# LRMPUT/PUTSLAM

Measured on AMD Instinct MI355X. Metric: frame-pairs/s (match+RANSAC+Kabsch), 640x480 @ 2000 kpts, higher is better.
Workload: dtype f32; 1 GPU; BASELINE configs[2]: TUM fr1/desk-style synthetic sequence, 500 frames = 499 frame pairs per step per GPU, 2000 kpts/frame, 256-bit descriptors, Hamming BF + cross-check -> depth filter -> H=4096 3-pt Umeyama hypotheses (fixed) scored with errorVersion 1 -> refit; inputs resident in HBM; kpts=2000, hypotheses=4096, world_size=1, force_dist=False, estimator=fixed, streams=4, join=end, submit=ps_batch_queue_submit: whole batches to the library's chains in turn, matcher_kernel=mfma-fused, score_kernel=fast, hw_queues=4, accepted_pairs=499

## Files before the change

### profiles/isa_mix.py

```python
#!/usr/bin/env python3
import json
import os
import re
import subprocess
import sys
import tempfile
from collections import Counter

ROOT = os.path.dirname(os.path.dirname(os.path.abspath(__file__)))
FLAGS = ["--offload-arch=gfx950", "-O3", "-ffp-contract=off", "-std=c++17", "-mllvm", "-amdgpu-mfma-vgpr-form",
         "-fno-slp-vectorize", "-mllvm", "-disable-vector-combine", "-S", "--cuda-device-only",
         "-I", os.path.join(ROOT, "include"), "-I", os.path.join(ROOT, "putslam_amd", "csrc")]


def asm_of(src, td, name):
    out = os.path.join(td, name)
    subprocess.check_call(["/opt/rocm/bin/hipcc"] + FLAGS + ["-o", out, src], stderr=subprocess.DEVNULL)
    return open(out).read()


def body_of(s, sym):
    a = s.index("\n" + sym)
    return s[a:s.index(".Lfunc_end", a)]


def blocks_of(body):
    parts = re.split(r"\n(\.LBB\d+_\d+:|; %bb\.\d+:)", body)
    return [(parts[i], parts[i + 1]) for i in range(1, len(parts), 2)]


def valu(txt):
    return Counter(re.sub(r"_e(32|64)$", "", l.split()[0]) for l in txt.split("\n") if l.strip().startswith("v_"))


def summary(c):
    n = sum(c.values())
    pk = sum(v for k, v in c.items() if k.startswith("v_pk_"))
    return {"valu": n, "packed": pk, "mix": dict(c)}


def main():
    out = {"source": "hipcc -S of putslam_amd/csrc/ps_capi.hip and profiles/microbench/prologue_isa.hip with the library's flags"}
    with tempfile.TemporaryDirectory() as td:
        s = asm_of(os.path.join(ROOT, "putslam_amd", "csrc", "ps_capi.hip"), td, "capi.s")
        pro = asm_of(os.path.join(ROOT, "profiles", "microbench", "prologue_isa.hip"), td, "pro.s")
    for mode in (1, 2):
        for kind, label in ((0, "stage0"), (1, "stage1")):
            bl = blocks_of(body_of(s, "_ZN5psdev20ps_ransac_score_fastILi%dELb1ELi%dELb0EE" % (mode, kind)))
            evals = [valu(t) for _, t in bl if "v_addc_co_u32" in t and t.count("v_pk_") >= 8]
            pre = [valu(t) for _, t in bl if "v_addc_co_u32" not in t and t.count("v_pk_") >= 12 and "ds_" not in t]
            e = {"unit": "(hypothesis, match) evaluation per wave"}
            if evals:
                per_block = max(1, evals[0]["v_addc_co_u32"])
                sm = summary(evals[0])
                e.update({"valu": sm["valu"] / per_block, "packed": sm["packed"] / per_block,
                          "mix": {k: v / per_block for k, v in sm["mix"].items()}})
                e["evaluations_per_block"] = per_block
                e["evaluation_blocks"] = len(evals)
            if pre and kind == 1:
                e["pretest"] = dict(summary(pre[0]), unit="TWO matches, one direction, per wave")
            out["ps_ransac_score_fast<%d> %s" % (mode, label)] = e
    for mode in (0, 4):
        bl = blocks_of(body_of(s, "_ZN5psdev22ps_ransac_score_euclidILi%dELi1ELb0EE" % mode))
        hot = [(t.count("clamp"), valu(t)) for _, t in bl if "clamp" in t]
        hot.sort(key=lambda x: -x[0])
        steps = hot[0][0]
        out["ps_ransac_score_euclid<%d>" % mode] = dict(summary(hot[0][1]), unit="block of %d packed steps = %d matches per wave" % (steps, 2 * steps),
                                                        valu_per_match=sum(hot[0][1].values()) / (2.0 * steps),
                                                        packed_per_match=sum(v for k, v in hot[0][1].items() if k.startswith("v_pk_")) / (2.0 * steps))
    for mode in (0, 1, 2, 4):
        bl = blocks_of(body_of(s, "_ZN5psdev15ps_ransac_scoreILi%dEE" % mode))
        loops = {}
        for n, t in bl:
            first = t.split("\n", 1)[0]
            m = re.search(r"Header=(BB\d+_\d+)", first)
            hdr = m.group(1) if m else (n.strip(".:L") if "Loop Header" in first else None)
            if hdr:
                loops.setdefault(hdr, []).append(t)
        best = max(loops.values(), key=lambda ts: sum(t.count("s_load_dwordx4") for t in ts))
        hot = Counter()
        for t in best:
            if "v_div_scale_f32" not in t and "v_cvt_f64_f32" not in t:
                hot += valu(t)
        per = max(1, "\n".join(best).count("s_load_dwordx4") // 2) if mode in (0, 4) else 1
        out["ps_ransac_score<%d>" % mode] = dict(summary(hot), unit="match loop body per wave (%d matches)" % per, valu_per_match=sum(hot.values()) / per)
    bl = blocks_of(body_of(s, "_ZN5psdev21ps_hamming_mfma_fusedILi4EE"))
    mf = max((t for _, t in bl), key=lambda t: t.count("v_mfma"))
    c = valu(mf)
    nm = sum(v for k, v in c.items() if k.startswith("v_mfma"))
    for k in [k for k in c if k.startswith("v_mfma")]:
        del c[k]
    out["ps_hamming_mfma_fused<4>"] = dict(summary(c), unit="query tile x 4 train tiles per wave (4096 distances)", mfma_per_unit=nm)
    bl = blocks_of(body_of(s, "_ZN5psdev13ps_hamming_nnILi2EE"))
    hb = max((t for _, t in bl), key=lambda t: t.count("v_bcnt"))
    c = valu(hb)
    out["ps_hamming_nn"] = dict(summary(c), unit="block of %d descriptor pairs per wave" % (c["v_bcnt_u32_b32"] // 8),
                                valu_per_pair=sum(c.values()) / (c["v_bcnt_u32_b32"] / 8.0))
    for sym in ("k_sample", "k_umeyama", "k_inverse"):
        bl = blocks_of(body_of(pro, sym + ":"))
        tot, loop = Counter(), Counter()
        for n, t in bl:
            c = valu(t)
            tot += c
            if "in Loop:" in t.split("\n", 1)[0] or "Loop Header" in t.split("\n", 1)[0]:
                loop += c
        full_div = tot["v_div_fixup_f32"]
        out["prologue " + sym] = {"static_valu": sum(tot.values()), "static_valu_in_loops": sum(loop.values()),
                                  "full_ieee_divisions": full_div, "reciprocal_chains": tot["v_rcp_f32"],
                                  "square_roots": tot["v_sqrt_f32"], "moves_and_selects": tot["v_mov_b32"] + tot["v_cndmask_b32"],
                                  "note": "static: both sides of every window check are in the count (short form AND the '/' fallback); "
                                          "the dynamic figure per wavefront is measured (sq_counters_by_grid.json, stage 0's models-only launch)"}
    with open(os.path.join(ROOT, "profiles", "isa_mix.json"), "w") as f:
        json.dump(out, f, indent=1)
    for k, v in out.items():
        if isinstance(v, dict):
            print(k, {a: b for a, b in v.items() if a not in ("mix", "note", "pretest")}, ("pretest %s" % {a: b for a, b in v["pretest"].items() if a != "mix"}) if "pretest" in v else "")


if __name__ == "__main__":
    main()
```

### putslam_amd/csrc/ps_matcher_mfma.h

```cpp
#pragma once

#include "ps_kernels.h"

namespace psdev {

typedef int v4i_t __attribute__((ext_vector_type(4)));
typedef int v8i_t __attribute__((ext_vector_type(8)));
typedef float v16f_t __attribute__((ext_vector_type(16)));

constexpr int kTileRows = 32;
constexpr int kTileU4 = 256;
constexpr int kWavesPerWG = kBlock / 64;

PS_HD constexpr uint32_t fp4_word(uint32_t w, int j, uint32_t sign = 0x88888888u, uint32_t fill = 0x66666666u)
{
    return (sign & (w << (3 - j))) | (~sign & fill);
}
constexpr bool fp4_word_checks(uint32_t w)
{
    for (int j = 0; j < 4; ++j) {
        const uint32_t o = fp4_word(w, j);
        if ((o & 0x77777777u) != 0x66666666u) return false;
        for (int i = 0; i < 8; ++i)
            if (((o >> (4 * i + 3)) & 1u) != ((w >> (4 * i + j)) & 1u)) return false;
    }
    return true;
}
constexpr bool fp4_single_bits_check()
{
    for (int b = 0; b < 32; ++b) {
        int hits = 0;
        for (int j = 0; j < 4; ++j)
            for (int i = 0; i < 8; ++i)
                if ((fp4_word(1u << b, j) >> (4 * i + 3)) & 1u) hits += (4 * i + j == b) ? 1 : 100;
        if (hits != 1 || !fp4_word_checks(1u << b) || !fp4_word_checks(~(1u << b))) return false;
    }
    return true;
}
static_assert(fp4_single_bits_check(), "every descriptor bit is the sign of exactly one nibble");
static_assert(fp4_word_checks(0u) && fp4_word_checks(0xFFFFFFFFu) && fp4_word_checks(0x80000001u) &&
                  fp4_word_checks(0xDEADBEEFu) && fp4_word_checks(0x01234567u) && fp4_word_checks(0xA5A5C3C3u) &&
                  fp4_word_checks(0x0F0F00FFu) && fp4_word_checks(0x13579BDFu),
              "fp4_word: sign of nibble i of dword j = bit 4 i + j, magnitude 0b110");
static_assert(fp4_word(0u, 0) == 0x66666666u && fp4_word(0xFFFFFFFFu, 2) == 0xEEEEEEEEu && fp4_word(0x10u, 0) == 0x000000E0u + 0x66666606u,
              "fp4_word: 0 -> +4.0, 1 -> -4.0");
PS_D v4i_t fp4_from_dword(uint32_t w)
{
    v4i_t r;
    r.x = (int)fp4_word(w, 0);
    r.y = (int)fp4_word(w, 1);
    r.z = (int)fp4_word(w, 2);
    r.w = (int)fp4_word(w, 3);
    return r;
}

PS_D int tile_row(int reg, int h) { return (reg & 3) + 8 * (reg >> 2) + 4 * h; }

__global__ __launch_bounds__(kBlock) void ps_expand_query_fp4(const uint32_t *__restrict__ desc,
                                                              const int32_t *__restrict__ nkpts,
                                                              const int32_t *__restrict__ pairs, int cap, int fstride, int tpf,
                                                              int chunks, uint4 *__restrict__ Xq,
                                                              uint32_t *__restrict__ keysInit)
{
    const int p = (int)(blockIdx.x / (unsigned)chunks), chunk = (int)(blockIdx.x % (unsigned)chunks);
    if (keysInit)
        for (int t = chunk * kBlock + threadIdx.x; t < cap; t += chunks * kBlock) keysInit[(size_t)p * cap + t] = kNoKey;
    const int fq = pairs[2 * p];
    const int nq = nkpts[fq];
    const uint32_t *__restrict__ q32 = desc + (size_t)fq * fstride;
    uint4 *__restrict__ out = Xq + (size_t)p * tpf * kTileU4;
    const int o = threadIdx.x, s = o >> 6, h = (o >> 5) & 1, r = o & 31;
    for (int tile = chunk; tile < tpf; tile += chunks) {
        const int row = tile * kTileRows + r;
        v4i_t e = {0, 0, 0, 0};
        if (row < nq) e = fp4_from_dword(q32[(size_t)row * 8 + 2 * s + h]);
        out[(size_t)tile * kTileU4 + o] = make_uint4((uint32_t)e.x, (uint32_t)e.y, (uint32_t)e.z, (uint32_t)e.w);
    }
}

PS_D v16f_t mfma_fp4(const v4i_t &a, const v4i_t &b, const v16f_t &c)
{
    const v8i_t a8 = __builtin_shufflevector(a, a, 0, 1, 2, 3, -1, -1, -1, -1);
    const v8i_t b8 = __builtin_shufflevector(b, b, 0, 1, 2, 3, -1, -1, -1, -1);
    return __builtin_amdgcn_mfma_scale_f32_32x32x64_f8f6f4(a8, b8, c, 4, 4, 0, 0, 0, 0);
}

PS_D v16f_t mfma_fp4s(const v4i_t &a, const v4i_t &b, const v16f_t &c)
{
    const v8i_t a8 = __builtin_shufflevector(a, a, 0, 1, 2, 3, -1, -1, -1, -1);
    const v8i_t b8 = __builtin_shufflevector(b, b, 0, 1, 2, 3, -1, -1, -1, -1);
    return __builtin_amdgcn_mfma_scale_f32_32x32x64_f8f6f4(a8, b8, c, 4, 4, 0, (int)0x88888888u, 0, (int)0x7F7F7F7Fu);
}

PS_D int fbits(float f) { return __builtin_bit_cast(int, f); }
PS_D int imax3(int a, int b, int c) { return max(max(a, b), c); }
PS_D int max16(const v16f_t &d)
{
    int m = imax3(fbits(d[0]), fbits(d[1]), fbits(d[2]));
    m = imax3(m, fbits(d[3]), fbits(d[4]));
    m = imax3(m, fbits(d[5]), fbits(d[6]));
    m = imax3(m, fbits(d[7]), fbits(d[8]));
    m = imax3(m, fbits(d[9]), fbits(d[10]));
    m = imax3(m, fbits(d[11]), fbits(d[12]));
    m = imax3(m, fbits(d[13]), fbits(d[14]));
    return max(m, fbits(d[15]));
}

constexpr float kMfmaNoRow = -1.0e30f;
constexpr int kMfmaBias = 8223;
constexpr float kMfmaBase = 8388608.0f;

#ifndef PS_MFMA_WAVES
#define PS_MFMA_WAVES 1
#endif
template <int TT>
__global__ __launch_bounds__(kBlock, PS_MFMA_WAVES) void ps_hamming_mfma(const uint32_t *__restrict__ desc,
                                                          const int32_t *__restrict__ nkpts,
                                                          const int32_t *__restrict__ pairs, int cap, int fstride, int tpf,
                                                          int groups, int qsplit, const uint4 *__restrict__ Xq,
                                                          uint32_t *__restrict__ keys)
{
    const unsigned perPair = (unsigned)(groups * qsplit);
    const unsigned L = xcd_remap(blockIdx.x, gridDim.x);
    const int p = (int)(L / perPair);
    const int inner = (int)(L - (unsigned)p * perPair);
    const int g = inner / qsplit, qs = inner - g * qsplit;
    const int fq = pairs[2 * p], ft = pairs[2 * p + 1];
    const int nq = nkpts[fq], nt = nkpts[ft];
    if (g * (kWavesPerWG * TT * kTileRows) >= nt) return;
    const int tid = threadIdx.x, lane = tid & 63, wave = tid >> 6;
    const int r = lane & 31, h = lane >> 5;
    const int tile0 = (g * kWavesPerWG + wave) * TT;
    const int nqTiles = (nq + kTileRows - 1) / kTileRows;
    const int T0 = (int)(((long long)nqTiles * qs) / qsplit), T1 = (int)(((long long)nqTiles * (qs + 1)) / qsplit);

    const uint32_t *__restrict__ t32 = desc + (size_t)ft * fstride;
    v4i_t B[TT][4];
#pragma unroll
    for (int i = 0; i < TT; ++i) {
        int t = (tile0 + i) * kTileRows + r;
        t = t < nt ? t : nt - 1;
#pragma unroll
        for (int s = 0; s < 4; ++s) B[i][s] = fp4_from_dword(t32[(size_t)t * 8 + 2 * s + h]);
    }
    v16f_t C;
#pragma unroll
    for (int reg = 0; reg < 16; ++reg) C[reg] = kMfmaBase + (float)(kMfmaBias - 4096 - tile_row(reg, h));
    int best[TT], bestT[TT];
#pragma unroll
    for (int i = 0; i < TT; ++i) {
        best[i] = 0;
        bestT[i] = 0;
    }

    const uint4 *__restrict__ xq = Xq + (size_t)p * tpf * kTileU4;
    uint4 an[4];
    if (T0 < T1) {
#pragma unroll
        for (int s = 0; s < 4; ++s) an[s] = xq[(size_t)T0 * kTileU4 + s * 64 + lane];
    }
    for (int T = T0; T < T1; ++T) {
        v4i_t A[4];
#pragma unroll
        for (int s = 0; s < 4; ++s) {
            A[s].x = (int)an[s].x; A[s].y = (int)an[s].y; A[s].z = (int)an[s].z; A[s].w = (int)an[s].w;
        }
        if (T + 1 < T1) {
#pragma unroll
            for (int s = 0; s < 4; ++s) an[s] = xq[(size_t)(T + 1) * kTileU4 + s * 64 + lane];
        }
        v16f_t Cin = C;
        if (T * kTileRows + kTileRows > nq) {
#pragma unroll
            for (int reg = 0; reg < 16; ++reg)
                if (T * kTileRows + tile_row(reg, h) >= nq) Cin[reg] = kMfmaNoRow;
        }
#pragma unroll
        for (int i = 0; i < TT; ++i) {
            v16f_t acc = mfma_fp4(A[0], B[i][0], Cin);
            acc = mfma_fp4(A[1], B[i][1], acc);
            acc = mfma_fp4(A[2], B[i][2], acc);
            acc = mfma_fp4(A[3], B[i][3], acc);
            const int m = max16(acc);
            if (m > (best[i] | 31)) {
                best[i] = m;
                bestT[i] = T;
            }
        }
    }
#pragma unroll
    for (int i = 0; i < TT; ++i) {
        const int t = (tile0 + i) * kTileRows + r;
        uint32_t key = kNoKey;
        if (best[i] > 0) {
            const int v = kMfmaBias - (best[i] & 0x7FFFFF);
            key = ((uint32_t)(v >> 5) << 16) | (uint32_t)(bestT[i] * kTileRows + (v & 31));
        }
        const uint32_t other = (uint32_t)__shfl_xor((int)key, 32, 64);
        key = other < key ? other : key;
        if (h == 0 && t < nt) {
            if (qsplit == 1)
                keys[(size_t)p * cap + t] = key;
            else
                atomicMin(&keys[(size_t)p * cap + t], key);
        }
    }
}

constexpr int kFuseChunk = 4;

template <int TT>
__global__ __launch_bounds__(kBlock, PS_MFMA_WAVES) void ps_hamming_mfma_fused(const uint32_t *__restrict__ desc,
                                                                const int32_t *__restrict__ nkpts,
                                                                const int32_t *__restrict__ pairs, int cap, int fstride, int tpf,
                                                                int groups, int qsplit, uint32_t *__restrict__ keys)
{
    __shared__ uint4 s_a[2][kFuseChunk][kTileU4];
    const unsigned perPair = (unsigned)(groups * qsplit);
    const unsigned L = xcd_remap(blockIdx.x, gridDim.x);
    const int p = (int)(L / perPair);
    const int inner = (int)(L - (unsigned)p * perPair);
    const int g = inner / qsplit, qs = inner - g * qsplit;
    const int fq = pairs[2 * p], ft = pairs[2 * p + 1];
    const int nq = nkpts[fq], nt = nkpts[ft];
    if (g * (kWavesPerWG * TT * kTileRows) >= nt) return;
    const int tid = threadIdx.x, lane = tid & 63, wave = tid >> 6;
    const int r = lane & 31, h = lane >> 5;
    const int tile0 = (g * kWavesPerWG + wave) * TT;
    const int nqTiles = (nq + kTileRows - 1) / kTileRows;
    const int T0 = (int)(((long long)nqTiles * qs) / qsplit), T1 = (int)(((long long)nqTiles * (qs + 1)) / qsplit);

    const uint32_t *__restrict__ t32 = desc + (size_t)ft * fstride;
    v4i_t B[TT][4];
#pragma unroll
    for (int i = 0; i < TT; ++i) {
        int t = (tile0 + i) * kTileRows + r;
        t = t < nt ? t : nt - 1;
#pragma unroll
        for (int s = 0; s < 4; ++s) B[i][s] = fp4_from_dword(t32[(size_t)t * 8 + 2 * s + h]);
    }
    v16f_t C;
#pragma unroll
    for (int reg = 0; reg < 16; ++reg) C[reg] = kMfmaBase + (float)((1 << 21) + 31 - tile_row(reg, h));
    int rel[TT];
#pragma unroll
    for (int i = 0; i < TT; ++i) rel[i] = 0;

    const uint32_t *__restrict__ q32 = desc + (size_t)fq * fstride;
    const int es = tid >> 6, eh = (tid >> 5) & 1, er = tid & 31;
    const int lastT = (nq & (kTileRows - 1)) ? nqTiles - 1 : -1;
    const bool hasPartial = lastT >= T0 && lastT < T1;
    const int Tm = hasPartial ? lastT : T1;
    const int nFull = (Tm - T0) / kFuseChunk;
    const int rem = (Tm - T0) - nFull * kFuseChunk;
    const int nTail = rem + (hasPartial ? 1 : 0);
    const int nChunks = nFull + (nTail > 0 ? 1 : 0);
    const uint32_t *__restrict__ qp = q32 + ((size_t)T0 * kTileRows + er) * 8 + 2 * es + eh;
    auto load_chunk = [&](int k, uint32_t (&W)[kFuseChunk]) {
        if (k < nFull) {
#pragma unroll
            for (int j = 0; j < kFuseChunk; ++j) W[j] = qp[j * (kTileRows * 8)];
            qp += kFuseChunk * kTileRows * 8;
        } else {
#pragma unroll
            for (int j = 0; j < kFuseChunk; ++j) {
                W[j] = 0;
                if (j < nTail && (T0 + nFull * kFuseChunk + j) * kTileRows + er < nq) W[j] = qp[j * (kTileRows * 8)];
            }
        }
    };
    uint32_t kSign = 0x88888888u, kFill = 0x66666666u;
    asm volatile("" : "+s"(kSign), "+v"(kFill));
    auto expand_chunk = [&](int buf, const uint32_t (&W)[kFuseChunk]) {
#pragma unroll
        for (int j = 0; j < kFuseChunk; ++j)
            s_a[buf][j][tid] = make_uint4(fp4_word(W[j], 0, kSign, kFill), fp4_word(W[j], 1, kSign, kFill),
                                          fp4_word(W[j], 2, kSign, kFill), fp4_word(W[j], 3, kSign, kFill));
    };
    auto tile_body = [&](const uint4 *__restrict__ tile, const v16f_t &Cin) {
        v4i_t A[4];
#pragma unroll
        for (int s = 0; s < 4; ++s) {
            const uint4 a = tile[s * 64 + lane];
            A[s].x = (int)a.x; A[s].y = (int)a.y; A[s].z = (int)a.z; A[s].w = (int)a.w;
        }
#pragma unroll
        for (int i = 0; i < TT; ++i) {
            v16f_t acc = mfma_fp4s(A[0], B[i][0], Cin);
            acc = mfma_fp4s(A[1], B[i][1], acc);
            acc = mfma_fp4s(A[2], B[i][2], acc);
            acc = mfma_fp4s(A[3], B[i][3], acc);
            int m = imax3(rel[i], fbits(acc[0]), fbits(acc[1]));
#pragma unroll
            for (int e = 2; e < 16; e += 2) m = imax3(m, fbits(acc[e]), fbits(acc[e + 1]));
            rel[i] = m + kTileRows;
        }
    };
    uint32_t W[kFuseChunk] = {0, 0, 0, 0};
    if (nChunks > 0) {
        load_chunk(0, W);
        expand_chunk(0, W);
    }
    if (nChunks > 1) load_chunk(1, W);
    __syncthreads();
    for (int k = 0; k < nFull; ++k) {
        expand_chunk((k + 1) & 1, W);
        if (k + 2 < nChunks) load_chunk(k + 2, W);
#pragma unroll 1
        for (int j = 0; j < kFuseChunk; ++j) tile_body(s_a[k & 1][j], C);
        __syncthreads();
    }
    if (nTail > 0) {
#pragma unroll 1
        for (int j = 0; j < rem; ++j) tile_body(s_a[nFull & 1][j], C);
        if (hasPartial) {
            v16f_t Cin = C;
#pragma unroll
            for (int reg = 0; reg < 16; ++reg)
                if (lastT * kTileRows + tile_row(reg, h) >= nq) Cin[reg] = kMfmaNoRow;
            tile_body(s_a[nFull & 1][rem], Cin);
        }
    }
    const int cEnd = 16352 - kTileRows * T1;
#pragma unroll
    for (int i = 0; i < TT; ++i) {
        const int t = (tile0 + i) * kTileRows + r;
        uint32_t key = kNoKey;
        if (rel[i] >= 0x4B000000) {
            const int d = (rel[i] + cEnd) & 0x7FFFFF;
            key = ((uint32_t)(256 - (d >> 14)) << 16) | (uint32_t)(16383 - (d & 0x3FFF));
        }
        const uint32_t other = (uint32_t)__shfl_xor((int)key, 32, 64);
        key = other < key ? other : key;
        if (h == 0 && t < nt) {
            if (qsplit == 1)
                keys[(size_t)p * cap + t] = key;
            else
                atomicMin(&keys[(size_t)p * cap + t], key);
        }
    }
}

}
```

Before: 599,600 frame-pairs/s.

## Double-buffer LDS tile reads in fused MFMA Hamming matcher and flatten max tree

```diff
diff --git a/profiles/isa_mix.py b/profiles/isa_mix.py
--- a/profiles/isa_mix.py
+++ b/profiles/isa_mix.py
@@ -90,7 +90,10 @@
     nm = sum(v for k, v in c.items() if k.startswith("v_mfma"))
     for k in [k for k in c if k.startswith("v_mfma")]:
         del c[k]
-    out["ps_hamming_mfma_fused<4>"] = dict(summary(c), unit="query tile x 4 train tiles per wave (4096 distances)", mfma_per_unit=nm)
+    tiles = max(1, nm // 16)
+    out["ps_hamming_mfma_fused<4>"] = dict(summary(c), unit="chunk of %d query tiles x 4 train tiles per wave (%d distances)" % (tiles, 4096 * tiles),
+                                           mfma_per_unit=nm, valu_per_query_tile=sum(c.values()) / float(tiles),
+                                           lds_reads_per_query_tile=mf.count("ds_read_b128") / float(tiles))
     bl = blocks_of(body_of(s, "_ZN5psdev13ps_hamming_nnILi2EE"))
     hb = max((t for _, t in bl), key=lambda t: t.count("v_bcnt"))
     c = valu(hb)
diff --git a/putslam_amd/csrc/ps_matcher_mfma.h b/putslam_amd/csrc/ps_matcher_mfma.h
--- a/putslam_amd/csrc/ps_matcher_mfma.h
+++ b/putslam_amd/csrc/ps_matcher_mfma.h
@@ -277,23 +277,28 @@
             s_a[buf][j][tid] = make_uint4(fp4_word(W[j], 0, kSign, kFill), fp4_word(W[j], 1, kSign, kFill),
                                           fp4_word(W[j], 2, kSign, kFill), fp4_word(W[j], 3, kSign, kFill));
     };
-    auto tile_body = [&](const uint4 *__restrict__ tile, const v16f_t &Cin) {
-        v4i_t A[4];
+    v4i_t A[2][4];
+    auto read_tile = [&](v4i_t (&dst)[4], const uint4 *__restrict__ tile) {
 #pragma unroll
         for (int s = 0; s < 4; ++s) {
             const uint4 a = tile[s * 64 + lane];
-            A[s].x = (int)a.x; A[s].y = (int)a.y; A[s].z = (int)a.z; A[s].w = (int)a.w;
-        }
+            dst[s].x = (int)a.x; dst[s].y = (int)a.y; dst[s].z = (int)a.z; dst[s].w = (int)a.w;
+        }
+        __builtin_amdgcn_sched_barrier(0);
+    };
+    auto tile_body = [&](const v4i_t (&a)[4], const v16f_t &Cin) {
 #pragma unroll
         for (int i = 0; i < TT; ++i) {
-            v16f_t acc = mfma_fp4s(A[0], B[i][0], Cin);
-            acc = mfma_fp4s(A[1], B[i][1], acc);
-            acc = mfma_fp4s(A[2], B[i][2], acc);
-            acc = mfma_fp4s(A[3], B[i][3], acc);
-            int m = imax3(rel[i], fbits(acc[0]), fbits(acc[1]));
-#pragma unroll
-            for (int e = 2; e < 16; e += 2) m = imax3(m, fbits(acc[e]), fbits(acc[e + 1]));
-            rel[i] = m + kTileRows;
+            v16f_t acc = mfma_fp4s(a[0], B[i][0], Cin);
+            acc = mfma_fp4s(a[1], B[i][1], acc);
+            acc = mfma_fp4s(a[2], B[i][2], acc);
+            acc = mfma_fp4s(a[3], B[i][3], acc);
+            int m[5];
+#pragma unroll
+            for (int e = 0; e < 5; ++e) m[e] = imax3(fbits(acc[3 * e]), fbits(acc[3 * e + 1]), fbits(acc[3 * e + 2]));
+            const int lo = imax3(m[0], m[1], m[2]), hi = imax3(m[3], m[4], fbits(acc[15]));
+            rel[i] = imax3(lo, hi, rel[i]) + kTileRows;
+            __builtin_amdgcn_sched_barrier(0);
         }
     };
     uint32_t W[kFuseChunk] = {0, 0, 0, 0};
@@ -303,22 +308,36 @@
     }
     if (nChunks > 1) load_chunk(1, W);
     __syncthreads();
+    if (nChunks > 0) read_tile(A[0], s_a[0][0]);
+    static_assert(kFuseChunk % 2 == 0, "a chunk's first tile always lands in A[0]");
+#pragma unroll 1
     for (int k = 0; k < nFull; ++k) {
         expand_chunk((k + 1) & 1, W);
         if (k + 2 < nChunks) load_chunk(k + 2, W);
-#pragma unroll 1
-        for (int j = 0; j < kFuseChunk; ++j) tile_body(s_a[k & 1][j], C);
-        __syncthreads();
+        __builtin_amdgcn_sched_barrier(0);
+#pragma unroll
+        for (int j = 0; j < kFuseChunk; ++j) {
+            if (j + 1 < kFuseChunk) {
+                read_tile(A[(j + 1) & 1], s_a[k & 1][j + 1]);
+            } else {
+                __syncthreads();
+                read_tile(A[0], s_a[(k + 1) & 1][0]);
+            }
+            tile_body(A[j & 1], C);
+        }
     }
     if (nTail > 0) {
-#pragma unroll 1
-        for (int j = 0; j < rem; ++j) tile_body(s_a[nFull & 1][j], C);
-        if (hasPartial) {
-            v16f_t Cin = C;
-#pragma unroll
-            for (int reg = 0; reg < 16; ++reg)
-                if (lastT * kTileRows + tile_row(reg, h) >= nq) Cin[reg] = kMfmaNoRow;
-            tile_body(s_a[nFull & 1][rem], Cin);
+#pragma unroll
+        for (int j = 0; j < kFuseChunk; ++j) {
+            if (j < nTail) {
+                if (j + 1 < kFuseChunk && j + 1 < nTail) read_tile(A[(j + 1) & 1], s_a[nFull & 1][j + 1]);
+                if (j + 1 == nTail && hasPartial) {
+#pragma unroll
+                    for (int reg = 0; reg < 16; ++reg)
+                        if (lastT * kTileRows + tile_row(reg, h) >= nq) C[reg] = kMfmaNoRow;
+                }
+                tile_body(A[j & 1], C);
+            }
         }
     }
     const int cEnd = 16352 - kTileRows * T1;
```

After: 602,300 frame-pairs/s (median of 6 runs). No clear change (+0.4%).
